# zserge/grayskull

Hardware: NVIDIA H100
Metric: Mpixels/s, gs_blur(r=5) + gs_sobel, 4096x4096 uint8 (higher is better)
Workload: dtype u8

## Files before the change

### grayskull_b200/csrc/box.cu

```cuda
#include <limits.h>
#include <string.h>

#include <type_traits>

#include "common.cuh"
#include "pairs.cuh"

namespace gsb {

constexpr int BX_STRIDE = 240;
constexpr int BX_PW = 64;
constexpr int BX_RMAX = 7;
constexpr int BX_WARPS = 4;
constexpr int BX_BH = 32;
constexpr int BX_TH = BX_WARPS * BX_BH;
constexpr int BX_THREADS = BX_WARPS * 32;
constexpr int BX_TILE_WORDS = BX_PW * (BX_TH + 2 * BX_RMAX);
constexpr int BX_SMEM = BX_TILE_WORDS * 4 + 226 * 8 + 16;

struct DivMagic {
  float inv, k;
};
__host__ __device__ inline DivMagic div_magic(unsigned count) {
  unsigned m = (16777216u + count - 1u) / count;
  DivMagic d;
  d.inv = (float)m * 5.9604644775390625e-08f;
  d.k = 8388608.0f - 0.5f * (float)m;
  return d;
}

__device__ __forceinline__ uint32_t div_lo(uint32_t t, float inv) {
  float fl;
  asm("{ .reg .b16 lo, hi; mov.b32 {lo, hi}, %1; cvt.rn.f32.u16 %0, lo; }" : "=f"(fl) : "r"(t));
  return __float_as_uint(__fmaf_rd(fl, inv, 8388608.0f));
}
__device__ __forceinline__ uint32_t div_hi(uint32_t t, float inv) {
  float fh;
  asm("{ .reg .b16 lo, hi; mov.b32 {lo, hi}, %1; cvt.rn.f32.u16 %0, hi; }" : "=f"(fh) : "r"(t));
  return __float_as_uint(__fmaf_rd(fh, inv, 8388608.0f));
}
__device__ __forceinline__ uint32_t pack4(uint32_t q0, uint32_t q1, uint32_t q2, uint32_t q3) {
  uint32_t a, b;
  asm("mad.lo.u32 %0, %1, 256, %2;" : "=r"(a) : "r"(q1), "r"(q0));
  asm("mad.lo.u32 %0, %1, 256, %2;" : "=r"(b) : "r"(q3), "r"(q2));
  return prmt(a, b, 0x5410);
}

template <int R>
__device__ __forceinline__ void window_sums(const uint32_t (&V)[12], uint32_t (&T)[4]) {
  constexpr bool ODD = (R & 1) != 0;
  constexpr int NP = ODD ? R : R + 1;
  constexpr int A0 = 8 - R;
  constexpr int M0 = ODD ? (A0 + 1) / 2 : A0 / 2;
  uint32_t ps = V[M0];
#pragma unroll
  for (int i = 1; i < NP; i++) ps += V[M0 + i];
#pragma unroll
  for (int p = 0; p < 4; p++) {
    const int m = M0 + p;
    uint32_t x16, tot;
    asm("mad.lo.u32 %0, %1, 0x10001, 0;" : "=r"(x16) : "r"(ps));
    x16 >>= 16;
    if (ODD) {
      const uint32_t edge = prmt(V[m - 1], V[m + NP], 0x5432);
      asm("mad.lo.u32 %0, %1, 0x10001, %2;" : "=r"(tot) : "r"(x16), "r"(edge));
      T[p] = tot;
    } else {
      asm("mad.lo.u32 %0, %1, 0x10001, 0;" : "=r"(tot) : "r"(x16));
      T[p] = tot - prmt(V[m + R], V[m], 0x5432);
    }
    if (p < 3) ps = ps + V[m + NP] - V[m];
  }
}

template <int R, bool INTERIOR>
__device__ __forceinline__ void box_quot(const uint32_t (&T)[4], const int (&cw)[8], int ch, const float2 *__restrict__ magic,
                                         uint32_t (&q)[8]) {
  constexpr int FULL = 2 * R + 1;
  constexpr float FINV = (float)((16777216u + FULL * FULL - 1u) / (FULL * FULL)) * 5.9604644775390625e-08f;
  if (INTERIOR) {
#pragma unroll
    for (int p = 0; p < 4; p++) {
      q[2 * p] = div_lo(T[p], FINV);
      q[2 * p + 1] = div_hi(T[p], FINV);
    }
  } else {
#pragma unroll
    for (int p = 0; p < 4; p++) {
      const float2 m0 = magic[cw[2 * p] * ch], m1 = magic[cw[2 * p + 1] * ch];
      q[2 * p] = div_lo(T[p], m0.x);
      q[2 * p + 1] = div_hi(T[p], m1.x);
    }
  }
}

template <int R, bool ADAPTIVE, bool INTERIOR>
__device__ __forceinline__ uint2 box_finish(const uint32_t (&T)[4], uint2 srcpx, const int (&cw)[8], int ch,
                                            const float2 *__restrict__ magic, int cparam) {
  uint32_t q[8];
  box_quot<R, INTERIOR>(T, cw, ch, magic, q);
  uint2 o;
  if (ADAPTIVE) {
    const int cc = max(-256, min(256, cparam));
    const uint32_t kc = (uint32_t)(cc + 0x7FFF) * 0x10001u;
    uint32_t e[4];
#pragma unroll
    for (int p = 0; p < 4; p++) {
      const uint32_t m = prmt(q[2 * p], q[2 * p + 1], 0x5410);
      const uint32_t sw = p < 2 ? srcpx.x : srcpx.y;
      const uint32_t sp = prmt(sw, 0, (p & 1) ? 0x4342 : 0x4140);
      e[p] = sp + kc - m;
    }
    o.x = prmt_raw(e[0], e[1], 0xFDB9);
    o.y = prmt_raw(e[2], e[3], 0xFDB9);
  } else {
    o.x = pack4(q[0], q[1], q[2], q[3]);
    o.y = pack4(q[4], q[5], q[6], q[7]);
  }
  return o;
}

__device__ __forceinline__ void unpack_pairs(uint2 v, uint32_t (&p)[4]) {
  p[0] = prmt(v.x, 0, 0x4140), p[1] = prmt(v.x, 0, 0x4342);
  p[2] = prmt(v.y, 0, 0x4140), p[3] = prmt(v.y, 0, 0x4342);
}

template <int R, bool ADAPTIVE>
__global__ void __launch_bounds__(BX_THREADS)
k_box_tma(const __grid_constant__ CUtensorMap tmap, uint8_t *__restrict__ dst, unsigned w, unsigned h, int cparam) {
  extern __shared__ __align__(128) unsigned char smem_raw[];
  uint32_t *tile = reinterpret_cast<uint32_t *>(smem_raw);
  float2 *magic = reinterpret_cast<float2 *>(smem_raw + BX_TILE_WORDS * 4);
  uint64_t &bar = *reinterpret_cast<uint64_t *>(smem_raw + BX_TILE_WORDS * 4 + 226 * 8);
  constexpr int ROWS = BX_TH + 2 * R;
  constexpr int FULL = 2 * R + 1;

  const unsigned frame = blockIdx.z;
  const int xb = (int)blockIdx.x * BX_STRIDE - 16;
  const int y0 = (int)blockIdx.y * BX_TH;
  const bool interior = xb + 8 - R >= 0 && xb + 8 + BX_STRIDE - 1 + R <= (int)w - 1 && y0 - R >= 0 &&
                        y0 + BX_TH - 1 + R <= (int)h - 1;
  if (threadIdx.x == 0) {
    mbar_init(&bar, 1);
    mbar_fence_init();
  }
  if (!interior) {
    for (unsigned c = threadIdx.x + 1; c < 226; c += BX_THREADS) {
      const DivMagic d = div_magic(c);
      magic[c] = make_float2(d.inv, d.k);
    }
  }
  __syncthreads();
  if (threadIdx.x == 0) {
    mbar_expect_tx(&bar, BX_PW * 4 * ROWS);
    tma_load_3d(tile, &tmap, xb / 4, y0 - R, frame, &bar);
  }

  const int warp = threadIdx.x >> 5, lane = threadIdx.x & 31;
  const int x = xb + 8 * lane;
  const int yb = y0 + warp * BX_BH;
  const bool out_lane = lane >= 1 && lane <= 30 && x >= 0 && x < (int)w;
  const uint32_t *in = tile + (warp * BX_BH) * BX_PW + 2 * lane;
  uint8_t *outp = dst + (size_t)frame * w * h + (size_t)yb * w + x;
  int cw[8];
#pragma unroll
  for (int j = 0; j < 8; j++) cw[j] = out_lane ? min(x + j + R, (int)w - 1) - max(x + j - R, 0) + 1 : 1;

  mbar_wait(&bar, 0);
  if (yb >= (int)h) return;

  uint32_t S[4] = {0, 0, 0, 0};
  uint32_t ring[2 * R + 1][4];
#pragma unroll
  for (int i = 0; i < 2 * R; i++) {
    uint32_t e[4];
    unpack_pairs(*reinterpret_cast<const uint2 *>(in + i * BX_PW), e);
#pragma unroll
    for (int k = 0; k < 4; k++) {
      S[k] += e[k];
      ring[i][k] = e[k];
    }
  }
  uint32_t L[4] = {0, 0, 0, 0};

  auto row_step = [&](int i, auto interior_tag) {
    constexpr bool INT = decltype(interior_tag)::value;
    uint32_t e[4];
    unpack_pairs(*reinterpret_cast<const uint2 *>(in + (i + 2 * R) * BX_PW), e);
#pragma unroll
    for (int k = 0; k < 4; k++) S[k] = S[k] + e[k] - L[k];
    if (INT) {
#pragma unroll
      for (int k = 0; k < 4; k++) {
        ring[(i + 2 * R) % (2 * R + 1)][k] = e[k];
        L[k] = ring[i % (2 * R + 1)][k];
      }
    } else {
      unpack_pairs(*reinterpret_cast<const uint2 *>(in + i * BX_PW), L);
    }
    uint32_t V[12], T[4];
#pragma unroll
    for (int k = 0; k < 4; k++) {
      V[4 + k] = S[k];
      V[k] = (R == 7 || k > 0) ? __shfl_up_sync(0xFFFFFFFFu, S[k], 1) : 0u;
      V[8 + k] = (R == 7 || k < 3) ? __shfl_down_sync(0xFFFFFFFFu, S[k], 1) : 0u;
    }
    window_sums<R>(V, T);
    uint2 srcpx = make_uint2(0, 0);
    if (ADAPTIVE) srcpx = *reinterpret_cast<const uint2 *>(in + (i + R) * BX_PW);
    int ch = FULL;
    if (!INT) {
      const int y = yb + i;
      ch = min(y + R, (int)h - 1) - max(y - R, 0) + 1;
    }
    const uint2 o = box_finish<R, ADAPTIVE, INT>(T, srcpx, cw, ch, magic, cparam);
    if (out_lane) st_cs_u2(outp, o);
    outp += w;
  };

  if (interior) {
#pragma unroll
    for (int i = 0; i < BX_BH; i++) row_step(i, std::true_type{});
  } else {
#pragma unroll 1
    for (int i = 0; i < BX_BH; i++) {
      if (yb + i >= (int)h) break;
      row_step(i, std::false_type{});
    }
  }
}



constexpr int BS_STRIDE = 240;
constexpr int BS_PW = 68;
constexpr int BS_STEPS = 8;
constexpr int BS_WARPS = 8;
constexpr int BS_THREADS = BS_WARPS * 32;
constexpr int BS_BROWS = 16 * BS_STEPS;
constexpr int BS_TH = BS_BROWS - 2;
constexpr int BS_IN_ROWS = BS_BROWS + 16;
constexpr int BS_STRIPS = 16;
constexpr int BS_IN_BYTES = BS_PW * 4 * BS_IN_ROWS;
constexpr int BS_BL_BYTES = BS_PW * 4 * BS_BROWS;
constexpr int BS_SMEM = BS_IN_BYTES + BS_BL_BYTES + 226 * 8 + 16;
static_assert(BS_IN_BYTES % 128 == 0, "the blurred tile follows the TMA destination");
static_assert(BS_TH % 16 == 14, "phase B: the last warp's band is 14 rows");

struct DivMagicTable {
  float2 e[226];
};
constexpr DivMagicTable make_div_magic_table() {
  DivMagicTable t{};
  for (unsigned c = 1; c < 226; c++) {
    const unsigned m = (16777216u + c - 1u) / c;
    t.e[c].x = (float)m * 5.9604644775390625e-08f;
    t.e[c].y = 8388608.0f - 0.5f * (float)m;
  }
  return t;
}
__constant__ DivMagicTable c_div_magic = make_div_magic_table();

__device__ __forceinline__ void mma_u8(uint32_t (&d)[4], const uint32_t (&a)[4], uint32_t b0, uint32_t b1, uint32_t c) {
  asm("mma.sync.aligned.m16n8k32.row.col.s32.u8.u8.s32 {%0, %1, %2, %3}, {%4, %5, %6, %7}, {%8, %9}, "
      "{%10, %10, %10, %10};"
      : "=r"(d[0]), "=r"(d[1]), "=r"(d[2]), "=r"(d[3])
      : "r"(a[0]), "r"(a[1]), "r"(a[2]), "r"(a[3]), "r"(b0), "r"(b1), "r"(c));
}
__device__ __forceinline__ uint32_t imad256(uint32_t hi, uint32_t lo) {
  uint32_t d;
  asm("mad.lo.u32 %0, %1, 256, %2;" : "=r"(d) : "r"(hi), "r"(lo));
  return d;
}

__device__ __forceinline__ void st_cs_7of8(uint8_t *p, uint2 v, bool left) {
  if (left) {
    asm volatile("st.global.cs.u8 [%0], %1;" ::"l"(p + 1), "r"(v.x >> 8) : "memory");
    asm volatile("st.global.cs.u16 [%0], %1;" ::"l"(p + 2), "r"(v.x >> 16) : "memory");
    asm volatile("st.global.cs.u32 [%0], %1;" ::"l"(p + 4), "r"(v.y) : "memory");
  } else {
    asm volatile("st.global.cs.u32 [%0], %1;" ::"l"(p), "r"(v.x) : "memory");
    asm volatile("st.global.cs.u16 [%0], %1;" ::"l"(p + 4), "r"(v.y) : "memory");
    asm volatile("st.global.cs.u8 [%0], %1;" ::"l"(p + 6), "r"(v.y >> 16) : "memory");
  }
}

template <int R>
__global__ void __launch_bounds__(BS_THREADS, 3)
k_blur_sobel_tma(const __grid_constant__ CUtensorMap tmap, uint8_t *__restrict__ dst, unsigned w, unsigned h) {
  extern __shared__ __align__(128) unsigned char smem_raw[];
  const uint32_t *in = reinterpret_cast<const uint32_t *>(smem_raw);
  unsigned char *bl = smem_raw + BS_IN_BYTES;
  float2 *magic = reinterpret_cast<float2 *>(smem_raw + BS_IN_BYTES + BS_BL_BYTES);
  uint64_t &bar = *reinterpret_cast<uint64_t *>(smem_raw + BS_IN_BYTES + BS_BL_BYTES + 226 * 8);
  constexpr int FULL = 2 * R + 1;
  constexpr unsigned FM = (16777216u + FULL * FULL - 1u) / (FULL * FULL);
  constexpr float FINV = (float)FM * 5.9604644775390625e-08f, FK = 8388608.0f - 0.5f * (float)FM;

  const unsigned frame = blockIdx.z;
  const int xb = (int)blockIdx.x * BS_STRIDE - 16;
  const int y0 = (int)blockIdx.y * BS_TH;
  const int Y = y0 - 1;
  if (threadIdx.x == 0) {
    mbar_init(&bar, 1);
    mbar_fence_init();
    mbar_expect_tx(&bar, BS_IN_BYTES);
    tma_load_3d(smem_raw, &tmap, xb / 4, Y - 8, frame, &bar);
  }
  if (Y - R < 0 || Y + BS_BROWS - 1 + R > (int)h - 1 || xb + 8 - R < 0 || xb + 8 + 16 * BS_STRIPS - 1 + R > (int)w - 1) {
    for (unsigned c = threadIdx.x + 1; c < 226; c += BS_THREADS) magic[c] = c_div_magic.e[c];
  }
  __syncthreads();

  const int warp = threadIdx.x >> 5, lane = threadIdx.x & 31;
  const int g = lane >> 2, t = lane & 3;
  uint32_t ah[4], av[4];
#pragma unroll
  for (int j = 0; j < 4; j++) {
    const int row = g + 8 * (j & 1), kb = 16 * (j >> 1) + 4 * t;
    uint32_t a = 0, v = 0;
#pragma unroll
    for (int i = 0; i < 4; i++) {
      const int k = kb + i;
      const int hrow = (k >> 4) * 16 + ((k >> 1) & 1) * 8 + 2 * ((k >> 2) & 3) + (k & 1);
      a |= (uint32_t)(abs(k - 8 - row) <= R) << (8 * i);
      v |= (uint32_t)(abs(hrow - 8 - row) <= R) << (8 * i);
    }
    ah[j] = a, av[j] = v;
  }

#pragma unroll
  for (int j = 0; j < 4; j++) asm("" : "+r"(ah[j]), "+r"(av[j]));
  float finv = FINV, fk = FK;
  asm("" : "+f"(finv), "+f"(fk));
  const bool rows_full = Y - R >= 0 && Y + BS_BROWS - 1 + R <= (int)h - 1;

  mbar_wait(&bar, 0);

  for (int s = warp; s < BS_STRIPS; s += BS_WARPS) {
    const int c0 = xb + 8 + 16 * s;
    if (c0 >= (int)w) break;
    const uint32_t *ip = in + g * BS_PW + 4 * s + t;
    unsigned char *bp = bl + g * (BS_PW * 4) + 16 * s + 2 * t;
    const bool cols_full = c0 - R >= 0 && c0 + 15 + R <= (int)w - 1;
    int cw[4];
#pragma unroll
    for (int j = 0; j < 4; j++) {
      const int c = c0 + 8 * (j >> 1) + 2 * t + (j & 1);
      cw[j] = max(min(c + R, (int)w - 1) - max(c - R, 0) + 1, 1);
    }
    auto make_pair = [&](int p, uint32_t (&o)[4]) {
      uint32_t P[4], Q[4];
      const uint32_t *r0 = ip + 16 * p * BS_PW, *r1 = r0 + 8 * BS_PW;
      mma_u8(P, ah, r0[0], r0[4], 0u);
      mma_u8(Q, ah, r1[0], r1[4], 0u);
#pragma unroll
      for (int hh = 0; hh < 2; hh++) {
        const uint32_t x = prmt(P[2 * hh], P[2 * hh + 1], 0x5140), y = prmt(Q[2 * hh], Q[2 * hh + 1], 0x5140);
        o[2 * hh] = prmt(x, y, 0x5410);
        o[2 * hh + 1] = prmt(x, y, 0x7632);
      }
    };
    uint32_t pa[4], pb[4];
    make_pair(0, pa);
    auto walk = [&](auto full_tag) {
      constexpr bool FULLW = decltype(full_tag)::value;
#pragma unroll
      for (int u = 0; u < BS_STEPS; u++) {
        const int yu = Y + 16 * u;
        if (yu >= (int)h) break;
        make_pair(u + 1, pb);
        int ch[2] = {FULL, FULL};
        if (!FULLW) {
#pragma unroll
          for (int e = 0; e < 2; e++) {
            const int y = yu + g + 8 * e;
            ch[e] = max(min(y + R, (int)h - 1) - max(y - R, 0) + 1, 1);
          }
        }
#pragma unroll
        for (int hh = 0; hh < 2; hh++) {
          uint32_t dl[4], dh[4];
          mma_u8(dl, av, pa[2 * hh], pb[2 * hh], 0x4B000000u);
          mma_u8(dh, av, pa[2 * hh + 1], pb[2 * hh + 1], 0u);
          uint32_t q[4];
#pragma unroll
          for (int j = 0; j < 4; j++) {
            float inv = finv, k = fk;
            if (!FULLW) {
              const float2 m = magic[cw[2 * hh + (j & 1)] * ch[j >> 1]];
              inv = m.x, k = m.y;
            }
            q[j] = __float_as_uint(__fmaf_rd(__uint_as_float(imad256(dh[j], dl[j])), inv, k));
          }
          unsigned char *o = bp + 16 * u * (BS_PW * 4) + 8 * hh;
          *reinterpret_cast<uint16_t *>(o) = (uint16_t)imad256(q[1], q[0]);
          *reinterpret_cast<uint16_t *>(o + 8 * (BS_PW * 4)) = (uint16_t)imad256(q[3], q[2]);
        }
#pragma unroll
        for (int j = 0; j < 4; j++) pa[j] = pb[j];
      }
    };
    if (cols_full && rows_full) walk(std::true_type{});
    else walk(std::false_type{});
  }
  __syncthreads();

  const int r0 = 16 * warp, nb = min(16, BS_TH - r0);
  const int x = xb + 16 + 8 * lane;
  const int yb = y0 + r0;
  const bool live = lane < 30 && x < (int)w;
  const bool edge_l = x == 0, edge_r = x + 8 == (int)w;
  const bool edge_warp = __any_sync(0xFFFFFFFFu, live && (edge_l || edge_r));
  if (!live || yb > (int)h - 2) return;
  const uint32_t *base = reinterpret_cast<const uint32_t *>(bl) + r0 * BS_PW + 2 * lane + 1;
  auto load_row = [&](int r) -> SobelRow {
    const uint32_t *p = base + r * BS_PW;
    const uint2 wm = *reinterpret_cast<const uint2 *>(p + 1);
    return sobel_row(split_pairs(p[0], wm.x, wm.y, p[3]));
  };
  uint8_t *outp = dst + (size_t)frame * w * h + (size_t)yb * w + x;
  SobelRow ra = load_row(0), rb = load_row(1);
  auto walk_full = [&](auto edge_tag) {
#pragma unroll
    for (int i = 0; i < 16; i++) {
      if (i >= BS_TH % 16 && i >= nb) break;
      const SobelRow rc = load_row(i + 2);
      const uint2 so = sobel_out(ra, rb, rc);
      if (!decltype(edge_tag)::value) {
        st_cs_u2(outp, so);
      } else {
        if (!edge_l && !edge_r) st_cs_u2(outp, so);
        if (edge_l) st_cs_7of8(outp, so, true);
        if (edge_r) st_cs_7of8(outp, so, false);
      }
      outp += w;
      ra = rb;
      rb = rc;
    }
  };
  if (yb >= 1 && yb + nb - 1 <= (int)h - 2) {
    if (edge_warp) walk_full(std::true_type{});
    else walk_full(std::false_type{});
  } else {
#pragma unroll 1
    for (int i = 0; i < nb; i++) {
      const int y = yb + i;
      if (y > (int)h - 2) break;
      const SobelRow rc = load_row(i + 2);
      if (y >= 1) {
        const uint2 so = sobel_out(ra, rb, rc);
        if (edge_l) st_cs_7of8(outp, so, true);
        else if (edge_r) st_cs_7of8(outp, so, false);
        else st_cs_u2(outp, so);
      }
      outp += w;
      ra = rb;
      rb = rc;
    }
  }
}

template <bool ADAPTIVE>
__global__ void __launch_bounds__(128)
k_box_wide(uint8_t *__restrict__ dst, const uint8_t *__restrict__ src, int w, int h, int r, int R8, int BH,
           int strips, int cparam, float minv, int fast_ok) {
  __shared__ uint32_t sp_all[4][8][64];
  const int warp = threadIdx.x >> 5, lane = threadIdx.x & 31;
  const int strip = (int)blockIdx.x * 4 + warp;
  if (strip >= strips) return;
  const int outw = 256 - 2 * R8;
  const int xs = strip * outw - R8;
  const int x0 = xs + 8 * lane;
  const int yb = (int)blockIdx.y * BH, ye = min(h, yb + BH);
  const uint8_t *frame = src + (size_t)blockIdx.z * w * h;
  uint8_t *out = dst + (size_t)blockIdx.z * w * h;
  const bool lane_in = x0 + 7 >= 0 && x0 < w;
  const bool out_lane = 8 * lane >= R8 && 8 * lane + 8 <= 256 - R8 && x0 < w && x0 + 7 >= 0;
  const int FULL = 2 * r + 1;
  const bool cols_full = x0 - r >= 0 && x0 + 7 + r <= w - 1;

  auto ldp = [&](const uint8_t *p, int y) -> uint2 {
    if (!lane_in || y < 0 || y >= h) return make_uint2(0u, 0u);
    uint32_t a = 0, b = 0;
#pragma unroll
    for (int k = 0; k < 4; k++) {
      if (x0 + k >= 0 && x0 + k < w) a |= (uint32_t)__ldg(p + k) << (8 * k);
      if (x0 + 4 + k >= 0 && x0 + 4 + k < w) b |= (uint32_t)__ldg(p + 4 + k) << (8 * k);
    }
    return make_uint2(a, b);
  };
  auto ld = [&](int y) -> uint2 { return ldp(frame + (ptrdiff_t)y * w + x0, y); };

  uint32_t S[4] = {0, 0, 0, 0};
#pragma unroll 4
  for (int yy = yb - r; yy <= yb + r; yy++) {
    uint32_t e[4];
    unpack_pairs(ld(yy), e);
#pragma unroll
    for (int k = 0; k < 4; k++) S[k] += e[k];
  }
  uint2 en = ld(yb + r + 1), lv = ld(yb - r), cen = make_uint2(0u, 0u);
  if (ADAPTIVE) cen = ld(yb);
  const uint8_t *p_en = frame + (ptrdiff_t)(yb + r + 2) * w + x0, *p_lv = frame + (ptrdiff_t)(yb + 1 - r) * w + x0;
  const uint8_t *p_cen = frame + (ptrdiff_t)(yb + 1) * w + x0;
  uint8_t *qo = out + (size_t)yb * w + x0;
  uint32_t (*sp)[64] = sp_all[warp];
  if (lane == 0) sp[7][15] = 0u;
  __syncwarp();
  const uint32_t *pA[8], *pB[8];
#pragma unroll
  for (int k = 0; k < 8; k++) {
    const int ca = k + r, cb = k - r - 1 + 128;
    pA[k] = &sp[0][0] + (ca & 7) * 64 + 16 + lane + (ca >> 3);
    pB[k] = &sp[0][0] + (cb & 7) * 64 + lane + (cb >> 3);
  }

  for (int y = yb; y < ye; y++) {
    const uint2 en2 = ldp(p_en, y + r + 2), lv2 = ldp(p_lv, y + 1 - r);
    uint2 cen2 = make_uint2(0u, 0u);
    if (ADAPTIVE) cen2 = ldp(p_cen, y + 1);
    p_en += w, p_lv += w, p_cen += w;
    uint32_t p[8];
#pragma unroll
    for (int k = 0; k < 4; k++) p[2 * k] = S[k] & 0xFFFFu, p[2 * k + 1] = S[k] >> 16;
#pragma unroll
    for (int k = 1; k < 8; k++) p[k] += p[k - 1];
    uint32_t incl = p[7];
#pragma unroll
    for (int o = 1; o < 32; o <<= 1) {
      const uint32_t t = __shfl_up_sync(0xFFFFFFFFu, incl, o);
      if (lane >= o) incl += t;
    }
    const uint32_t excl = incl - p[7];
    __syncwarp();
#pragma unroll
    for (int k = 0; k < 8; k++) sp[k][16 + lane] = p[k] + excl;
    __syncwarp();
    if (out_lane) {
      uint32_t W[8];
#pragma unroll
      for (int k = 0; k < 8; k++) W[k] = *pA[k] - *pB[k];
      const int ch = min(y + r, h - 1) - max(y - r, 0) + 1;
      uint32_t q[8];
      if (fast_ok && cols_full && ch == FULL) {
#pragma unroll
        for (int k = 0; k < 8; k++) q[k] = __float_as_uint(__fmaf_rd((float)W[k], minv, 8388608.0f)) & 0xFFu;
      } else {
#pragma unroll
        for (int k = 0; k < 8; k++) {
          const int x = x0 + k;
          const int cw = min(x + r, w - 1) - max(x - r, 0) + 1;
          q[k] = __float2uint_rd(__fdiv_rn((float)W[k], (float)(cw * ch)));
        }
      }
      if (ADAPTIVE) {
#pragma unroll
        for (int k = 0; k < 8; k++) {
          const int sv = (int)(((k < 4 ? cen.x : cen.y) >> (8 * (k & 3))) & 0xFFu);
          q[k] = sv > (int)(q[k] - (unsigned)cparam) ? 255u : 0u;
        }
      }
      uint2 o;
      o.x = q[0] | (q[1] << 8) | (q[2] << 16) | (q[3] << 24);
      o.y = q[4] | (q[5] << 8) | (q[6] << 16) | (q[7] << 24);
#pragma unroll
      for (int k = 0; k < 8; k++)
        if (x0 + k >= 0 && x0 + k < w) qo[k] = (uint8_t)((k < 4 ? o.x : o.y) >> (8 * (k & 3)));
    }
    qo += w;
    uint32_t e[4], l[4];
    unpack_pairs(en, e);
    unpack_pairs(lv, l);
#pragma unroll
    for (int k = 0; k < 4; k++) S[k] = S[k] + e[k] - l[k];
    en = en2, lv = lv2, cen = cen2;
  }
}

constexpr int BM_PITCH = 130;
constexpr int BM_WARP_WORDS = 32 * BM_PITCH + 8;
constexpr int BM_SMEM = BM_WARP_WORDS * 4;

__device__ const uint2 bm_zero8 = {0u, 0u};

__device__ __forceinline__ uint32_t pack4_alu(uint32_t q0, uint32_t q1, uint32_t q2, uint32_t q3) {
  return prmt(prmt(q0, q1, 0x0040), prmt(q2, q3, 0x0040), 0x5410);
}

template <bool SUB>
__device__ __forceinline__ uint32_t dp2a_half(uint32_t acc, uint32_t word, int half) {
  uint32_t d;
  if (!SUB) {
    if (half) asm("dp2a.lo.u32.u32 %0, %1, 0x0100, %2;" : "=r"(d) : "r"(word), "r"(acc));
    else asm("dp2a.lo.u32.u32 %0, %1, 0x0001, %2;" : "=r"(d) : "r"(word), "r"(acc));
  } else {
    if (half) asm("dp2a.lo.u32.s32 %0, %1, 0xFF00, %2;" : "=r"(d) : "r"(word), "r"(acc));
    else asm("dp2a.lo.u32.s32 %0, %1, 0x00FF, %2;" : "=r"(d) : "r"(word), "r"(acc));
  }
  return d;
}
__device__ __forceinline__ void unpack_pairs_alt(uint2 v, uint32_t (&p)[4]) {
  p[0] = v.x & 0x00FF00FFu, p[1] = prmt(v.x, 0, 0x4341);
  p[2] = v.y & 0x00FF00FFu, p[3] = prmt(v.y, 0, 0x4341);
}
template <bool SUB>
__device__ __forceinline__ uint32_t dp2a_elem(uint32_t acc, uint2 a, uint2 b, int idx) {
  const uint2 g = idx < 4 ? a : b;
  return dp2a_half<SUB>(acc, (idx & 1) ? g.y : g.x, (idx >> 1) & 1);
}

template <int RM, bool ADAPTIVE>
// ... 202 lines not shown
    if (out_lane) {
      const uint32_t *orow = cs + 2 + ((8 * lane - R8) >> 2);
      uint8_t *qo = out + (size_t)yc * w + x0;
      const uint8_t *qc = frame + (size_t)yc * w + x0;
      const unsigned wu = (unsigned)w;
      auto put_row = [&](int j) {
        uint2 o = *reinterpret_cast<const uint2 *>(orow + j * BM_PITCH);
        if (ADAPTIVE) {
          const uint2 sp = __ldg(reinterpret_cast<const uint2 *>(qc + (size_t)j * wu));
          const uint32_t e0 = prmt(sp.x, 0, 0x4140) + kc - prmt(o.x, 0, 0x4140);
          const uint32_t e1 = prmt(sp.x, 0, 0x4342) + kc - prmt(o.x, 0, 0x4342);
          const uint32_t e2 = prmt(sp.y, 0, 0x4140) + kc - prmt(o.y, 0, 0x4140);
          const uint32_t e3 = prmt(sp.y, 0, 0x4342) + kc - prmt(o.y, 0, 0x4342);
          o.x = prmt_raw(e0, e1, 0xFDB9);
          o.y = prmt_raw(e2, e3, 0xFDB9);
        }
        st_cs_u2(qo + (size_t)j * wu, o);
      };
      if (nrows == 32) {
        if (ADAPTIVE) {
#pragma unroll
          for (int j0 = 0; j0 < 32; j0 += 8) {
            uint2 sp[8];
#pragma unroll
            for (int j = 0; j < 8; j++) sp[j] = __ldg(reinterpret_cast<const uint2 *>(qc + (size_t)(j0 + j) * wu));
#pragma unroll
            for (int j = 0; j < 8; j++) {
              uint2 o = *reinterpret_cast<const uint2 *>(orow + (j0 + j) * BM_PITCH);
              const uint32_t e0 = prmt(sp[j].x, 0, 0x4140) + kc - prmt(o.x, 0, 0x4140);
              const uint32_t e1 = prmt(sp[j].x, 0, 0x4342) + kc - prmt(o.x, 0, 0x4342);
              const uint32_t e2 = prmt(sp[j].y, 0, 0x4140) + kc - prmt(o.y, 0, 0x4140);
              const uint32_t e3 = prmt(sp[j].y, 0, 0x4342) + kc - prmt(o.y, 0, 0x4342);
              st_cs_u2(qo + (size_t)(j0 + j) * wu, make_uint2(prmt_raw(e0, e1, 0xFDB9), prmt_raw(e2, e3, 0xFDB9)));
            }
          }
        } else {
#pragma unroll
          for (int j = 0; j < 32; j++) put_row(j);
        }
      } else {
#pragma unroll 1
        for (int j = 0; j < nrows; j++) put_row(j);
      }
    }
  }
}

static bool box_wide_magic(unsigned count, float *minv) {
  int lg = 0;
  while ((2u << lg) <= count) lg++;
  const int k = 23 + lg;
  const unsigned long long m = ((1ull << k) + count - 1) / count;
  if (m >= (1ull << 24)) return false;
  const unsigned long long e = m * count - (1ull << k);
  if (255ull * count * e >= (1ull << k)) return false;
  *minv = ldexpf((float)m, -k);
  return true;
}

template <bool ADAPTIVE>
__global__ void k_box_generic(uint8_t *__restrict__ dst, const uint8_t *__restrict__ src, unsigned w,
                              unsigned h, unsigned n, unsigned r, int cparam) {
  const unsigned x = blockIdx.x * blockDim.x + threadIdx.x;
  const unsigned y = blockIdx.y * blockDim.y + threadIdx.y;
  if (x >= w || y >= h) return;
  const unsigned xa = x > r ? x - r : 0, xb = min(x + (unsigned long long)r, (unsigned long long)w - 1);
  const unsigned ya = y > r ? y - r : 0, yb = min(y + (unsigned long long)r, (unsigned long long)h - 1);
  const unsigned count = (xb - xa + 1) * (yb - ya + 1);
  for (unsigned f = blockIdx.z; f < n; f += gridDim.z) {
    const uint8_t *s = src + (size_t)f * w * h;
    unsigned sum = 0;
    for (unsigned yy = ya; yy <= yb; yy++)
      for (unsigned xx = xa; xx <= xb; xx++) sum += s[(size_t)yy * w + xx];
    const unsigned mean = sum / count;
    uint8_t v;
    if (ADAPTIVE) v = ((int)s[(size_t)y * w + x] > (int)(mean - (unsigned)cparam)) ? 255 : 0;
    else v = (uint8_t)mean;
    dst[(size_t)f * w * h + (size_t)y * w + x] = v;
  }
}

template <bool ADAPTIVE>
static int launch_box(uint8_t *dst, const uint8_t *src, unsigned w, unsigned h, unsigned n, unsigned r,
                      int cparam, cudaStream_t s) {
  if (n == 0) return 0;
  const bool lane_c_ok = !ADAPTIVE || cparam > INT_MIN + 255;
  CUtensorMap tmap;
  if (lane_c_ok && r >= 1 && r <= BX_RMAX && tma_ok(src, w) && tma_ok(dst, w) &&
      n <= 65535u && make_tmap_u8frames(&tmap, src, w, h, n, BX_PW, BX_TH + 2 * r)) {
    static decltype(&k_box_tma<1, ADAPTIVE>) const box_tma_fn[BX_RMAX] = {
        k_box_tma<1, ADAPTIVE>, k_box_tma<2, ADAPTIVE>, k_box_tma<3, ADAPTIVE>, k_box_tma<4, ADAPTIVE>,
        k_box_tma<5, ADAPTIVE>, k_box_tma<6, ADAPTIVE>, k_box_tma<7, ADAPTIVE>};
    const unsigned tiles_x = (w + 8 + BX_STRIDE - 1) / BX_STRIDE, tiles_y = (h + BX_TH - 1) / BX_TH;
    GSB_ASSERT(tiles_y <= 65535u);
    GSB_LAUNCH(box_tma_fn[r - 1], dim3(tiles_x, tiles_y, n), BX_THREADS, BX_SMEM, s, tmap, dst, w, h, cparam);
    return 0;
  }
  if (r >= 1 && r <= 120 && !force_generic() && n <= 65535u && w < (1u << 30) && h < (1u << 30)) {
    const int R8 = (int)((r + 7) / 8 * 8), outw = 256 - 2 * R8;
    const int strips = (int)((w + outw - 1) / outw);
    const long long want = (long long)sm_count() * 24;
    long long bands = (want + (long long)strips * n - 1) / ((long long)strips * n);
    const long long max_bands = ((long long)h + (4 * (long long)r > 32 ? 4 * (long long)r : 32) - 1) / (4 * (long long)r > 32 ? 4 * (long long)r : 32);
    if (bands > max_bands) bands = max_bands;
    if (bands < 1) bands = 1;
    int BH = (int)((h + bands - 1) / bands);
    const unsigned gy = (h + BH - 1) / BH;
    GSB_ASSERT(gy <= 65535u);
    float minv = 0.0f;
    const int fast_ok = (r <= 63 && box_wide_magic((2 * r + 1) * (2 * r + 1), &minv)) ? 1 : 0;
    const bool aligned = w % 8 == 0 && reinterpret_cast<uintptr_t>(src) % 8 == 0 && reinterpret_cast<uintptr_t>(dst) % 8 == 0;
    dim3 grid((strips + 3) / 4, gy, n);
    if (aligned && lane_c_ok) {
      const long long four_waves = (long long)sm_count() * 13 * 4;
      BH = 32;
      for (int cand = 128; cand >= 32; cand >>= 1)
        if ((long long)strips * ((h + cand - 1) / cand) * n >= four_waves || cand == 32) { BH = cand; break; }
      while (BH < 4 * (int)r && BH < 256) BH <<= 1;
      const long long warps = (long long)strips * ((h + BH - 1) / BH);
      GSB_ASSERT(warps < (1ll << 31));
      grid = dim3((unsigned)warps, 1, n);
      CUtensorMap pmap;
      const int use_tpf = make_tmap_u8frames(&pmap, src, w, h, n, 72, 32) ? 1 : 0;
      if (!use_tpf) memset(&pmap, 0, sizeof(pmap));
      static decltype(&k_box_mid<0, ADAPTIVE>) const box_mid_fn[4] = {k_box_mid<0, ADAPTIVE>, k_box_mid<1, ADAPTIVE>,
                                                                      k_box_mid<2, ADAPTIVE>, k_box_mid<3, ADAPTIVE>};
      GSB_LAUNCH(box_mid_fn[r & 3], grid, 32, BM_SMEM, s, pmap, use_tpf, dst, src, (int)w, (int)h, (int)r, R8, BH, strips,
                 cparam, minv, fast_ok);
      return 0;
    }
    GSB_LAUNCH(k_box_wide<ADAPTIVE>, grid, 128, 0, s, dst, src, (int)w, (int)h, (int)r, R8, BH, strips, cparam, minv, fast_ok);
    return 0;
  }
  dim3 block(32, 8), grid((w + 31) / 32, (h + 7) / 8, n < 65535u ? n : 65535u);
  GSB_LAUNCH(k_box_generic<ADAPTIVE>, grid, block, 0, s, dst, src, w, h, n, r, cparam);
  return 0;
}

}

extern "C" {
int gs_b200_blur_sobel_batch(uint8_t *dst, const uint8_t *src, unsigned w, unsigned h, unsigned n, unsigned radius,
                             gs_b200_stream st) {
  GSB_ASSERT(dst && src && w > 0 && h > 0);
  cudaStream_t s = static_cast<cudaStream_t>(st);
  if (n == 0 || w < 3 || h < 3) return 0;
  CUtensorMap tmap;
  if (radius >= 1 && radius <= gsb::BX_RMAX && gsb::tma_ok(src, w) && gsb::tma_ok(dst, w) && n <= 65535u &&
      gsb::make_tmap_u8frames(&tmap, src, w, h, n, gsb::BS_PW, gsb::BS_IN_ROWS)) {
    static decltype(&gsb::k_blur_sobel_tma<1>) const blur_sobel_fn[gsb::BX_RMAX] = {
        gsb::k_blur_sobel_tma<1>, gsb::k_blur_sobel_tma<2>, gsb::k_blur_sobel_tma<3>, gsb::k_blur_sobel_tma<4>,
        gsb::k_blur_sobel_tma<5>, gsb::k_blur_sobel_tma<6>, gsb::k_blur_sobel_tma<7>};
    const unsigned tiles_x = (w + gsb::BS_STRIDE - 1) / gsb::BS_STRIDE, tiles_y = (h + gsb::BS_TH - 1) / gsb::BS_TH;
    GSB_ASSERT(tiles_y <= 65535u);
    GSB_LAUNCH(blur_sobel_fn[radius - 1], dim3(tiles_x, tiles_y, n), gsb::BS_THREADS, gsb::BS_SMEM, s, tmap, dst, w, h);
    return 0;
  }
  uint8_t *tmp = static_cast<uint8_t *>(gsb::workspace(s, gsb::WS_STAGE_FUSED, (size_t)w * h * n));
  if (!tmp) return (int)cudaErrorMemoryAllocation;
  int rc = gs_b200_blur_batch(tmp, src, w, h, n, radius, st);
  if (rc) return rc;
  return gs_b200_sobel_batch(dst, tmp, w, h, n, st);
}
int gs_b200_blur_batch(uint8_t *dst, const uint8_t *src, unsigned w, unsigned h, unsigned n,
                       unsigned radius, gs_b200_stream s) {
  GSB_ASSERT(dst && src && w > 0 && h > 0);
  return gsb::launch_box<false>(dst, src, w, h, n, radius, 0, static_cast<cudaStream_t>(s));
}
int gs_b200_adaptive_threshold_batch(uint8_t *dst, const uint8_t *src, unsigned w, unsigned h,
                                     unsigned n, unsigned radius, int c, gs_b200_stream s) {
  GSB_ASSERT(dst && src && w > 0 && h > 0);
  return gsb::launch_box<true>(dst, src, w, h, n, radius, c, static_cast<cudaStream_t>(s));
}
}
```

### grayskull_b200/csrc/common.cuh

```cuda
#pragma once
#include <cuda.h>
#include <cuda_fp16.h>
#include <cuda_runtime.h>
#include <stdint.h>
#include <stdio.h>
#include <stdlib.h>

#include <utility>

#include "../../include/grayskull_b200.h"

namespace gsb {

int record_error(cudaError_t e, const char *file, int line);
bool force_generic();
int sm_count();

#define GSB_CHECK(expr)                                                        \
  do {                                                                         \
    cudaError_t gsb_e_ = (expr);                                               \
    if (gsb_e_ != cudaSuccess) return gsb::record_error(gsb_e_, __FILE__, __LINE__); \
  } while (0)

int opt_in_smem(const void *k, size_t smem, const char *file, int line);
int launched(const char *file, int line);

#ifdef __CUDACC__
template <class... P, class... A>
int launch(const char *file, int line, void (*k)(P...), dim3 grid, dim3 block, size_t smem, cudaStream_t s,
           A &&...a) {
  if (smem)
    if (int rc = opt_in_smem(reinterpret_cast<const void *>(k), smem, file, line)) return rc;
  k<<<grid, block, smem, s>>>(std::forward<A>(a)...);
  return launched(file, line);
}
#define GSB_LAUNCH(...)                                         \
  do {                                                          \
    int gsb_rc_ = gsb::launch(__FILE__, __LINE__, __VA_ARGS__); \
    if (gsb_rc_) return gsb_rc_;                                \
  } while (0)
#endif

#define GSB_ASSERT(cond)                                \
  do {                                                  \
    if (!(cond)) {                                      \
      fprintf(stderr, "Assertion failed: %s\n", #cond); \
      abort();                                          \
    }                                                   \
  } while (0)

void *workspace(cudaStream_t s, int slot, size_t bytes);

enum { WS_INTEGRAL = 0, WS_FAST_A, WS_FAST_B, WS_ORB_A, WS_ORB_B, WS_LBP_A, WS_LBP_B, WS_LBP_C,
       WS_STAGE_A, WS_STAGE_B, WS_STAGE_C, WS_STAGE_D, WS_HIST, WS_STAGE_FUSED, WS_BLOB_A, WS_BLOB_B, WS_BLOB_C, WS_MORPH, WS_SLOTS };

bool make_tmap_u8frames(CUtensorMap *m, const void *base, unsigned w, unsigned h, unsigned n,
                        unsigned box_words, unsigned box_rows);
bool make_tmap_u32frames(CUtensorMap *m, const void *base, unsigned w, unsigned h, unsigned n,
                         unsigned box_w, unsigned box_h);
inline bool tma_ok(const void *p, unsigned w) {
  return !force_generic() && (w % 16u) == 0 && (reinterpret_cast<uintptr_t>(p) % 16u) == 0;
}

#ifdef __CUDACC__
__device__ __forceinline__ uint32_t smem_u32(const void *p) {
  return static_cast<uint32_t>(__cvta_generic_to_shared(p));
}
__device__ __forceinline__ void mbar_init(uint64_t *bar, unsigned count) {
  asm volatile("mbarrier.init.shared::cta.b64 [%0], %1;" ::"r"(smem_u32(bar)), "r"(count) : "memory");
}
__device__ __forceinline__ void mbar_fence_init() {
  asm volatile("fence.mbarrier_init.release.cluster;" ::: "memory");
  asm volatile("fence.proxy.async.shared::cta;" ::: "memory");
}
__device__ __forceinline__ void mbar_expect_tx(uint64_t *bar, unsigned bytes) {
  asm volatile("mbarrier.arrive.expect_tx.shared::cta.b64 _, [%0], %1;" ::"r"(smem_u32(bar)), "r"(bytes)
               : "memory");
}
__device__ __forceinline__ void mbar_wait(uint64_t *bar, unsigned parity) {
  asm volatile(
      "{\n"
      ".reg .pred p;\n"
      "WAIT_%=:\n"
      "mbarrier.try_wait.parity.shared::cta.b64 p, [%0], %1;\n"
      "@p bra DONE_%=;\n"
      "bra WAIT_%=;\n"
      "DONE_%=:\n"
      "}" ::"r"(smem_u32(bar)),
      "r"(parity)
      : "memory");
}
__device__ __forceinline__ void tma_load_3d(void *smem_dst, const CUtensorMap *map, int c0, int c1,
                                            int c2, uint64_t *bar) {
  asm volatile(
      "cp.async.bulk.tensor.3d.shared::cluster.global.mbarrier::complete_tx::bytes"
      " [%0], [%1, {%2, %3, %4}], [%5];" ::"r"(smem_u32(smem_dst)),
      "l"(reinterpret_cast<uint64_t>(map)), "r"(c0), "r"(c1), "r"(c2), "r"(smem_u32(bar))
      : "memory");
}

__device__ __forceinline__ uint32_t prmt(uint32_t a, uint32_t b, uint32_t sel) {
  return __byte_perm(a, b, sel);
}
__device__ __forceinline__ uint32_t prmt_raw(uint32_t a, uint32_t b, uint32_t sel) {
  uint32_t d;
  asm("prmt.b32 %0, %1, %2, %3;" : "=r"(d) : "r"(a), "r"(b), "r"(sel));
  return d;
}
__device__ __forceinline__ void st_cs_u2(void *p, uint2 v) {
  asm volatile("st.global.cs.v2.u32 [%0], {%1, %2};" ::"l"(p), "r"(v.x), "r"(v.y) : "memory");
}
#endif

}
```

Measured before the change: 1.242 million.

## Make fused blur+sobel kernel persistent with atomic tile scheduler and TMA prefetch

The one-CTA-per-tile grid becomes a persistent grid of one CTA per SM, each holding three independent 256-thread workers with their own staging buffers and mbarriers. Each worker pulls its next tile from a global atomic counter and issues that tile's TMA load once its blur phase has finished with the input stage. The load then overlaps the sobel phase of the current tile. This removes block launch and prologue costs and hides load latency, in exchange for atomics, named-barrier syncs, and a per-launch counter memset.

Result: faster. 1.275 million (median of 6 runs) (+2.7%).

```diff
diff --git a/grayskull_b200/csrc/box.cu b/grayskull_b200/csrc/box.cu
--- a/grayskull_b200/csrc/box.cu
+++ b/grayskull_b200/csrc/box.cu
@@ -1,6 +1,7 @@
 #include <limits.h>
 #include <string.h>
 
+#include <algorithm>
 #include <type_traits>
 
 #include "common.cuh"
@@ -237,14 +238,21 @@
 constexpr int BS_STEPS = 8;
 constexpr int BS_WARPS = 8;
 constexpr int BS_THREADS = BS_WARPS * 32;
+constexpr int BS_WORKERS = 3;
+constexpr int BS_CTA_THREADS = BS_WORKERS * BS_THREADS;
 constexpr int BS_BROWS = 16 * BS_STEPS;
 constexpr int BS_TH = BS_BROWS - 2;
 constexpr int BS_IN_ROWS = BS_BROWS + 16;
 constexpr int BS_STRIPS = 16;
 constexpr int BS_IN_BYTES = BS_PW * 4 * BS_IN_ROWS;
 constexpr int BS_BL_BYTES = BS_PW * 4 * BS_BROWS;
-constexpr int BS_SMEM = BS_IN_BYTES + BS_BL_BYTES + 226 * 8 + 16;
-static_assert(BS_IN_BYTES % 128 == 0, "the blurred tile follows the TMA destination");
+constexpr int BS_BL_OFF = BS_WORKERS * BS_IN_BYTES;
+constexpr int BS_MAGIC_OFF = BS_BL_OFF + BS_WORKERS * BS_BL_BYTES;
+constexpr int BS_BAR_OFF = BS_MAGIC_OFF + 226 * 8;
+constexpr int BS_NEXT_OFF = BS_BAR_OFF + BS_WORKERS * 8;
+constexpr int BS_SMEM = BS_NEXT_OFF + BS_WORKERS * 4;
+static_assert(BS_IN_BYTES % 128 == 0 && BS_BL_BYTES % 128 == 0, "TMA destinations stay 128-byte aligned");
+static_assert(BS_SMEM <= 232448, "the per-block shared-memory opt-in of an H100");
 static_assert(BS_TH % 16 == 14, "phase B: the last warp's band is 14 rows");
 
 struct DivMagicTable {
@@ -285,34 +293,62 @@
   }
 }
 
+struct DivU31 {
+  unsigned d, m, s;
+};
+inline DivU31 div_u31(unsigned d) {
+  unsigned l = 0;
+  while ((1ull << l) < d) l++;
+  return {d, (unsigned)(((1ull << (31 + l)) + d - 1) / d), 31 + l};
+}
+__device__ __forceinline__ unsigned div_u31(unsigned n, const DivU31 &q) {
+  return (unsigned)(((unsigned long long)n * q.m) >> q.s);
+}
+
+struct BsTile {
+  int xb, y0;
+  unsigned frame;
+};
+__device__ __forceinline__ BsTile bs_tile(unsigned v, const DivU31 &tx, const DivU31 &ty) {
+  const unsigned vy = div_u31(v, tx), frame = div_u31(vy, ty);
+  return {(int)(v - vy * tx.d) * BS_STRIDE - 16, (int)(vy - frame * ty.d) * BS_TH, frame};
+}
+
+__device__ __forceinline__ void bs_worker_sync(int id) {
+  asm volatile("bar.sync %0, %1;" ::"r"(id), "n"(BS_THREADS) : "memory");
+}
+
 template <int R>
-__global__ void __launch_bounds__(BS_THREADS, 3)
-k_blur_sobel_tma(const __grid_constant__ CUtensorMap tmap, uint8_t *__restrict__ dst, unsigned w, unsigned h) {
+__global__ void __launch_bounds__(BS_CTA_THREADS, 1)
+k_blur_sobel_tma(const __grid_constant__ CUtensorMap tmap, uint8_t *__restrict__ dst, unsigned w, unsigned h,
+                 unsigned tiles, DivU31 tx, DivU31 ty, unsigned *__restrict__ counter) {
   extern __shared__ __align__(128) unsigned char smem_raw[];
-  const uint32_t *in = reinterpret_cast<const uint32_t *>(smem_raw);
-  unsigned char *bl = smem_raw + BS_IN_BYTES;
-  float2 *magic = reinterpret_cast<float2 *>(smem_raw + BS_IN_BYTES + BS_BL_BYTES);
-  uint64_t &bar = *reinterpret_cast<uint64_t *>(smem_raw + BS_IN_BYTES + BS_BL_BYTES + 226 * 8);
+  const int worker = threadIdx.x / BS_THREADS, wt = threadIdx.x % BS_THREADS;
+  unsigned char *stage = smem_raw + worker * BS_IN_BYTES;
+  const uint32_t *in = reinterpret_cast<const uint32_t *>(stage);
+  unsigned char *bl = smem_raw + BS_BL_OFF + worker * BS_BL_BYTES;
+  float2 *magic = reinterpret_cast<float2 *>(smem_raw + BS_MAGIC_OFF);
+  uint64_t *bar = reinterpret_cast<uint64_t *>(smem_raw + BS_BAR_OFF) + worker;
+  unsigned *next = reinterpret_cast<unsigned *>(smem_raw + BS_NEXT_OFF) + worker;
   constexpr int FULL = 2 * R + 1;
   constexpr unsigned FM = (16777216u + FULL * FULL - 1u) / (FULL * FULL);
   constexpr float FINV = (float)FM * 5.9604644775390625e-08f, FK = 8388608.0f - 0.5f * (float)FM;
 
-  const unsigned frame = blockIdx.z;
-  const int xb = (int)blockIdx.x * BS_STRIDE - 16;
-  const int y0 = (int)blockIdx.y * BS_TH;
-  const int Y = y0 - 1;
-  if (threadIdx.x == 0) {
-    mbar_init(&bar, 1);
+  const unsigned first = BS_WORKERS * blockIdx.x + worker;
+  auto load = [&](unsigned v) {
+    const BsTile tl = bs_tile(v, tx, ty);
+    mbar_expect_tx(bar, BS_IN_BYTES);
+    tma_load_3d(stage, &tmap, tl.xb / 4, tl.y0 - 9, (int)tl.frame, bar);
+  };
+  if (wt == 0 && first < tiles) {
+    mbar_init(bar, 1);
     mbar_fence_init();
-    mbar_expect_tx(&bar, BS_IN_BYTES);
-    tma_load_3d(smem_raw, &tmap, xb / 4, Y - 8, frame, &bar);
-  }
-  if (Y - R < 0 || Y + BS_BROWS - 1 + R > (int)h - 1 || xb + 8 - R < 0 || xb + 8 + 16 * BS_STRIPS - 1 + R > (int)w - 1) {
-    for (unsigned c = threadIdx.x + 1; c < 226; c += BS_THREADS) magic[c] = c_div_magic.e[c];
-  }
+    load(first);
+  }
+  for (unsigned c = threadIdx.x + 1; c < 226; c += BS_CTA_THREADS) magic[c] = c_div_magic.e[c];
   __syncthreads();
 
-  const int warp = threadIdx.x >> 5, lane = threadIdx.x & 31;
+  const int warp = wt >> 5, lane = wt & 31;
   const int g = lane >> 2, t = lane & 3;
   uint32_t ah[4], av[4];
 #pragma unroll
@@ -333,131 +369,149 @@
   for (int j = 0; j < 4; j++) asm("" : "+r"(ah[j]), "+r"(av[j]));
   float finv = FINV, fk = FK;
   asm("" : "+f"(finv), "+f"(fk));
-  const bool rows_full = Y - R >= 0 && Y + BS_BROWS - 1 + R <= (int)h - 1;
-
-  mbar_wait(&bar, 0);
-
-  for (int s = warp; s < BS_STRIPS; s += BS_WARPS) {
-    const int c0 = xb + 8 + 16 * s;
-    if (c0 >= (int)w) break;
-    const uint32_t *ip = in + g * BS_PW + 4 * s + t;
-    unsigned char *bp = bl + g * (BS_PW * 4) + 16 * s + 2 * t;
-    const bool cols_full = c0 - R >= 0 && c0 + 15 + R <= (int)w - 1;
-    int cw[4];
-#pragma unroll
-    for (int j = 0; j < 4; j++) {
-      const int c = c0 + 8 * (j >> 1) + 2 * t + (j & 1);
-      cw[j] = max(min(c + R, (int)w - 1) - max(c - R, 0) + 1, 1);
-    }
-    auto make_pair = [&](int p, uint32_t (&o)[4]) {
-      uint32_t P[4], Q[4];
-      const uint32_t *r0 = ip + 16 * p * BS_PW, *r1 = r0 + 8 * BS_PW;
-      mma_u8(P, ah, r0[0], r0[4], 0u);
-      mma_u8(Q, ah, r1[0], r1[4], 0u);
-#pragma unroll
-      for (int hh = 0; hh < 2; hh++) {
-        const uint32_t x = prmt(P[2 * hh], P[2 * hh + 1], 0x5140), y = prmt(Q[2 * hh], Q[2 * hh + 1], 0x5140);
-        o[2 * hh] = prmt(x, y, 0x5410);
-        o[2 * hh + 1] = prmt(x, y, 0x7632);
+
+#pragma unroll 1
+  for (unsigned v = first, parity = 0; v < tiles; parity ^= 1) {
+    const BsTile tl = bs_tile(v, tx, ty);
+    const int xb = tl.xb, y0 = tl.y0;
+    const unsigned frame = tl.frame;
+    const int Y = y0 - 1;
+    const bool rows_full = Y - R >= 0 && Y + BS_BROWS - 1 + R <= (int)h - 1;
+    mbar_wait(bar, parity);
+
+    for (int s = warp; s < BS_STRIPS; s += BS_WARPS) {
+      const int c0 = xb + 8 + 16 * s;
+      if (c0 >= (int)w) break;
+      const uint32_t *ip = in + g * BS_PW + 4 * s + t;
+      unsigned char *bp = bl + g * (BS_PW * 4) + 16 * s + 2 * t;
+      const bool cols_full = c0 - R >= 0 && c0 + 15 + R <= (int)w - 1;
+      int cw[4];
+#pragma unroll
+      for (int j = 0; j < 4; j++) {
+        const int c = c0 + 8 * (j >> 1) + 2 * t + (j & 1);
+        cw[j] = max(min(c + R, (int)w - 1) - max(c - R, 0) + 1, 1);
       }
-    };
-    uint32_t pa[4], pb[4];
-    make_pair(0, pa);
-    auto walk = [&](auto full_tag) {
-      constexpr bool FULLW = decltype(full_tag)::value;
-#pragma unroll
-      for (int u = 0; u < BS_STEPS; u++) {
-        const int yu = Y + 16 * u;
-        if (yu >= (int)h) break;
-        make_pair(u + 1, pb);
-        int ch[2] = {FULL, FULL};
-        if (!FULLW) {
-#pragma unroll
-          for (int e = 0; e < 2; e++) {
-            const int y = yu + g + 8 * e;
-            ch[e] = max(min(y + R, (int)h - 1) - max(y - R, 0) + 1, 1);
+      auto make_pair = [&](int p, uint32_t (&o)[4]) {
+        uint32_t P[4], Q[4];
+        const uint32_t *r0 = ip + 16 * p * BS_PW, *r1 = r0 + 8 * BS_PW;
+        mma_u8(P, ah, r0[0], r0[4], 0u);
+        mma_u8(Q, ah, r1[0], r1[4], 0u);
+#pragma unroll
+        for (int hh = 0; hh < 2; hh++) {
+          const uint32_t x = prmt(P[2 * hh], P[2 * hh + 1], 0x5140), y = prmt(Q[2 * hh], Q[2 * hh + 1], 0x5140);
+          o[2 * hh] = prmt(x, y, 0x5410);
+          o[2 * hh + 1] = prmt(x, y, 0x7632);
+        }
+      };
+      uint32_t pa[4], pb[4];
+      make_pair(0, pa);
+      auto walk = [&](auto full_tag) {
+        constexpr bool FULLW = decltype(full_tag)::value;
+#pragma unroll
+        for (int u = 0; u < BS_STEPS; u++) {
+          const int yu = Y + 16 * u;
+          if (yu >= (int)h) break;
+          make_pair(u + 1, pb);
+          int ch[2] = {FULL, FULL};
+          if (!FULLW) {
+#pragma unroll
+            for (int e = 0; e < 2; e++) {
+              const int y = yu + g + 8 * e;
+              ch[e] = max(min(y + R, (int)h - 1) - max(y - R, 0) + 1, 1);
+            }
           }
-        }
-#pragma unroll
-        for (int hh = 0; hh < 2; hh++) {
-          uint32_t dl[4], dh[4];
-          mma_u8(dl, av, pa[2 * hh], pb[2 * hh], 0x4B000000u);
-          mma_u8(dh, av, pa[2 * hh + 1], pb[2 * hh + 1], 0u);
-          uint32_t q[4];
-#pragma unroll
-          for (int j = 0; j < 4; j++) {
-            float inv = finv, k = fk;
-            if (!FULLW) {
-              const float2 m = magic[cw[2 * hh + (j & 1)] * ch[j >> 1]];
-              inv = m.x, k = m.y;
+#pragma unroll
+          for (int hh = 0; hh < 2; hh++) {
+            uint32_t dl[4], dh[4];
+            mma_u8(dl, av, pa[2 * hh], pb[2 * hh], 0x4B000000u);
+            mma_u8(dh, av, pa[2 * hh + 1], pb[2 * hh + 1], 0u);
+            uint32_t q[4];
+#pragma unroll
+            for (int j = 0; j < 4; j++) {
+              float inv = finv, k = fk;
+              if (!FULLW) {
+                const float2 m = magic[cw[2 * hh + (j & 1)] * ch[j >> 1]];
+                inv = m.x, k = m.y;
+              }
+              q[j] = __float_as_uint(__fmaf_rd(__uint_as_float(imad256(dh[j], dl[j])), inv, k));
             }
-            q[j] = __float_as_uint(__fmaf_rd(__uint_as_float(imad256(dh[j], dl[j])), inv, k));
+            unsigned char *o = bp + 16 * u * (BS_PW * 4) + 8 * hh;
+            *reinterpret_cast<uint16_t *>(o) = (uint16_t)imad256(q[1], q[0]);
+            *reinterpret_cast<uint16_t *>(o + 8 * (BS_PW * 4)) = (uint16_t)imad256(q[3], q[2]);
           }
-          unsigned char *o = bp + 16 * u * (BS_PW * 4) + 8 * hh;
-          *reinterpret_cast<uint16_t *>(o) = (uint16_t)imad256(q[1], q[0]);
-          *reinterpret_cast<uint16_t *>(o + 8 * (BS_PW * 4)) = (uint16_t)imad256(q[3], q[2]);
-        }
-#pragma unroll
-        for (int j = 0; j < 4; j++) pa[j] = pb[j];
+#pragma unroll
+          for (int j = 0; j < 4; j++) pa[j] = pb[j];
+        }
+      };
+      if (cols_full && rows_full) walk(std::true_type{});
+      else walk(std::false_type{});
+    }
+    bs_worker_sync(1 + worker);
+    if (wt == 0) {
+      const unsigned nv = BS_WORKERS * gridDim.x + atomicAdd(counter, 1u);
+      *next = nv;
+      if (nv < tiles) {
+        asm volatile("fence.proxy.async.shared::cta;" ::: "memory");
+        load(nv);
       }
-    };
-    if (cols_full && rows_full) walk(std::true_type{});
-    else walk(std::false_type{});
-  }
-  __syncthreads();
-
-  const int r0 = 16 * warp, nb = min(16, BS_TH - r0);
-  const int x = xb + 16 + 8 * lane;
-  const int yb = y0 + r0;
-  const bool live = lane < 30 && x < (int)w;
-  const bool edge_l = x == 0, edge_r = x + 8 == (int)w;
-  const bool edge_warp = __any_sync(0xFFFFFFFFu, live && (edge_l || edge_r));
-  if (!live || yb > (int)h - 2) return;
-  const uint32_t *base = reinterpret_cast<const uint32_t *>(bl) + r0 * BS_PW + 2 * lane + 1;
-  auto load_row = [&](int r) -> SobelRow {
-    const uint32_t *p = base + r * BS_PW;
-    const uint2 wm = *reinterpret_cast<const uint2 *>(p + 1);
-    return sobel_row(split_pairs(p[0], wm.x, wm.y, p[3]));
-  };
-  uint8_t *outp = dst + (size_t)frame * w * h + (size_t)yb * w + x;
-  SobelRow ra = load_row(0), rb = load_row(1);
-  auto walk_full = [&](auto edge_tag) {
-#pragma unroll
-    for (int i = 0; i < 16; i++) {
-      if (i >= BS_TH % 16 && i >= nb) break;
-      const SobelRow rc = load_row(i + 2);
-      const uint2 so = sobel_out(ra, rb, rc);
-      if (!decltype(edge_tag)::value) {
-        st_cs_u2(outp, so);
+    }
+
+    const int r0 = 16 * warp, nb = min(16, BS_TH - r0);
+    const int x = xb + 16 + 8 * lane;
+    const int yb = y0 + r0;
+    const bool live = lane < 30 && x < (int)w;
+    const bool edge_l = x == 0, edge_r = x + 8 == (int)w;
+    const bool edge_warp = __any_sync(0xFFFFFFFFu, live && (edge_l || edge_r));
+    if (live && yb <= (int)h - 2) {
+      const uint32_t *base = reinterpret_cast<const uint32_t *>(bl) + r0 * BS_PW + 2 * lane + 1;
+      auto load_row = [&](int r) -> SobelRow {
+        const uint32_t *p = base + r * BS_PW;
+        const uint2 wm = *reinterpret_cast<const uint2 *>(p + 1);
+        return sobel_row(split_pairs(p[0], wm.x, wm.y, p[3]));
+      };
+      uint8_t *outp = dst + (size_t)frame * w * h + (size_t)yb * w + x;
+      SobelRow ra = load_row(0), rb = load_row(1);
+      auto walk_full = [&](auto edge_tag) {
+#pragma unroll
+        for (int i = 0; i < 16; i++) {
+          if (i >= BS_TH % 16 && i >= nb) break;
+          const SobelRow rc = load_row(i + 2);
+          const uint2 so = sobel_out(ra, rb, rc);
+          if (!decltype(edge_tag)::value) {
+            st_cs_u2(outp, so);
+          } else {
+            if (!edge_l && !edge_r) st_cs_u2(outp, so);
+            if (edge_l) st_cs_7of8(outp, so, true);
+            if (edge_r) st_cs_7of8(outp, so, false);
+          }
+          outp += w;
+          ra = rb;
+          rb = rc;
+        }
+      };
+      if (yb >= 1 && yb + nb - 1 <= (int)h - 2) {
+        if (edge_warp) walk_full(std::true_type{});
+        else walk_full(std::false_type{});
       } else {
-        if (!edge_l && !edge_r) st_cs_u2(outp, so);
-        if (edge_l) st_cs_7of8(outp, so, true);
-        if (edge_r) st_cs_7of8(outp, so, false);
+#pragma unroll 1
+        for (int i = 0; i < nb; i++) {
+          const int y = yb + i;
+          if (y > (int)h - 2) break;
+          const SobelRow rc = load_row(i + 2);
+          if (y >= 1) {
+            const uint2 so = sobel_out(ra, rb, rc);
+            if (edge_l) st_cs_7of8(outp, so, true);
+            else if (edge_r) st_cs_7of8(outp, so, false);
+            else st_cs_u2(outp, so);
+          }
+          outp += w;
+          ra = rb;
+          rb = rc;
+        }
       }
-      outp += w;
-      ra = rb;
-      rb = rc;
-    }
-  };
-  if (yb >= 1 && yb + nb - 1 <= (int)h - 2) {
-    if (edge_warp) walk_full(std::true_type{});
-    else walk_full(std::false_type{});
-  } else {
-#pragma unroll 1
-    for (int i = 0; i < nb; i++) {
-      const int y = yb + i;
-      if (y > (int)h - 2) break;
-      const SobelRow rc = load_row(i + 2);
-      if (y >= 1) {
-        const uint2 so = sobel_out(ra, rb, rc);
-        if (edge_l) st_cs_7of8(outp, so, true);
-        else if (edge_r) st_cs_7of8(outp, so, false);
-        else st_cs_u2(outp, so);
-      }
-      outp += w;
-      ra = rb;
-      rb = rc;
-    }
+    }
+    bs_worker_sync(1 + worker);
+    v = *next;
   }
 }
 
@@ -966,8 +1020,15 @@
         gsb::k_blur_sobel_tma<1>, gsb::k_blur_sobel_tma<2>, gsb::k_blur_sobel_tma<3>, gsb::k_blur_sobel_tma<4>,
         gsb::k_blur_sobel_tma<5>, gsb::k_blur_sobel_tma<6>, gsb::k_blur_sobel_tma<7>};
     const unsigned tiles_x = (w + gsb::BS_STRIDE - 1) / gsb::BS_STRIDE, tiles_y = (h + gsb::BS_TH - 1) / gsb::BS_TH;
-    GSB_ASSERT(tiles_y <= 65535u);
-    GSB_LAUNCH(blur_sobel_fn[radius - 1], dim3(tiles_x, tiles_y, n), gsb::BS_THREADS, gsb::BS_SMEM, s, tmap, dst, w, h);
+    const unsigned long long tiles = (unsigned long long)tiles_x * tiles_y * n;
+    GSB_ASSERT(tiles < (1ull << 31));
+    const unsigned ctas = (unsigned)std::min<unsigned long long>(
+        (unsigned long long)gsb::sm_count(), (tiles + gsb::BS_WORKERS - 1) / gsb::BS_WORKERS);
+    unsigned *counter = static_cast<unsigned *>(gsb::workspace(s, gsb::WS_TILE_COUNTER, sizeof(unsigned)));
+    if (!counter) return (int)cudaErrorMemoryAllocation;
+    GSB_CHECK(cudaMemsetAsync(counter, 0, sizeof(unsigned), s));
+    GSB_LAUNCH(blur_sobel_fn[radius - 1], ctas, gsb::BS_CTA_THREADS, gsb::BS_SMEM, s, tmap, dst, w, h,
+               (unsigned)tiles, gsb::div_u31(tiles_x), gsb::div_u31(tiles_y), counter);
     return 0;
   }
   uint8_t *tmp = static_cast<uint8_t *>(gsb::workspace(s, gsb::WS_STAGE_FUSED, (size_t)w * h * n));
diff --git a/grayskull_b200/csrc/common.cuh b/grayskull_b200/csrc/common.cuh
--- a/grayskull_b200/csrc/common.cuh
+++ b/grayskull_b200/csrc/common.cuh
@@ -52,7 +52,7 @@
 void *workspace(cudaStream_t s, int slot, size_t bytes);
 
 enum { WS_INTEGRAL = 0, WS_FAST_A, WS_FAST_B, WS_ORB_A, WS_ORB_B, WS_LBP_A, WS_LBP_B, WS_LBP_C,
-       WS_STAGE_A, WS_STAGE_B, WS_STAGE_C, WS_STAGE_D, WS_HIST, WS_STAGE_FUSED, WS_BLOB_A, WS_BLOB_B, WS_BLOB_C, WS_MORPH, WS_SLOTS };
+       WS_STAGE_A, WS_STAGE_B, WS_STAGE_C, WS_STAGE_D, WS_HIST, WS_STAGE_FUSED, WS_BLOB_A, WS_BLOB_B, WS_BLOB_C, WS_MORPH, WS_TILE_COUNTER, WS_SLOTS };
 
 bool make_tmap_u8frames(CUtensorMap *m, const void *base, unsigned w, unsigned h, unsigned n,
                         unsigned box_words, unsigned box_rows);
```
